# jirsat/wavenets

Measured on AMD Instinct MI355X. Metric: audio samples/sec (training step, 16 kHz mu-law), higher is better.
Workload: dtype f32 (fp16 hi|lo split operands, fp32 accumulate)

## Files before the change

wavenets_amd/csrc/wn_split16.h:

```cpp
#pragma once
#include <hip/hip_fp16.h>

#include "wn_kernels.h"

namespace wn_split16 {

typedef _Float16 h8 __attribute__((ext_vector_type(8)));
typedef _Float16 h4 __attribute__((ext_vector_type(4)));

__device__ __forceinline__ f32x16 mfma16(h8 a, h8 b, f32x16 c) {
  return __builtin_amdgcn_mfma_f32_32x32x16_f16(a, b, c, 0, 0, 0);
}

__device__ __forceinline__ void mfma3(const h8& a_hi, const h8& a_lo, const h8& b_hi, const h8& b_lo, f32x16& acc) {
  acc = mfma16(a_lo, b_hi, acc);
  acc = mfma16(a_hi, b_lo, acc);
  acc = mfma16(a_hi, b_hi, acc);
}

__device__ __forceinline__ void split8(const float (&v)[8], h8& hi, h8& lo) {
#pragma unroll
  for (int e = 0; e < 8; ++e) {
    const _Float16 h = (_Float16)v[e];
    hi[e] = h;
    lo[e] = (_Float16)(v[e] - (float)h);
  }
}
__device__ __forceinline__ void split8(const f32x4& q0, const f32x4& q1, h8& hi, h8& lo) {
  const float v[8] = {q0.x, q0.y, q0.z, q0.w, q1.x, q1.y, q1.z, q1.w};
  split8(v, hi, lo);
}
__device__ __forceinline__ void split4(const f32x4& q, h4& hi, h4& lo) {
  const float v[4] = {q.x, q.y, q.z, q.w};
#pragma unroll
  for (int e = 0; e < 4; ++e) {
    const _Float16 h = (_Float16)v[e];
    hi[e] = h;
    lo[e] = (_Float16)(v[e] - (float)h);
  }
}

__device__ __forceinline__ void split8s(const float (&v)[8], float s, h8& hi, h8& lo) {
#pragma unroll
  for (int e = 0; e < 8; ++e) {
    const _Float16 h = (_Float16)(v[e] * s);
    hi[e] = h;
    lo[e] = (_Float16)__builtin_fmaf(v[e], s, -(float)h);
  }
}
__device__ __forceinline__ void split8s(const f32x4& q0, const f32x4& q1, float s, h8& hi, h8& lo) {
  const float v[8] = {q0.x, q0.y, q0.z, q0.w, q1.x, q1.y, q1.z, q1.w};
  split8s(v, s, hi, lo);
}
__device__ __forceinline__ void split4s(const f32x4& q, float s, h4& hi, h4& lo) {
  const float v[4] = {q.x, q.y, q.z, q.w};
#pragma unroll
  for (int e = 0; e < 4; ++e) {
    const _Float16 h = (_Float16)(v[e] * s);
    hi[e] = h;
    lo[e] = (_Float16)__builtin_fmaf(v[e], s, -(float)h);
  }
}

__device__ __forceinline__ void pow2_scale(float m, float& sc, float& inv) {
  float s = 1.0f, i = 1.0f;
  if (m > 0.f && m < 3.0e38f) {
    int e;
    (void)frexpf(m, &e);
    e = max(-100, min(100, e));
    s = ldexpf(1.0f, -e);
    i = ldexpf(1.0f, e);
  }
  sc = s;
  inv = i;
}

__device__ __forceinline__ f32x4 ldg4(const float* p) { return *(const __attribute__((address_space(1))) f32x4*)(p); }
__device__ __forceinline__ f32x4 ldg4(const __attribute__((address_space(1))) char* p) {
  return *(const __attribute__((address_space(1))) f32x4*)p;
}

__device__ __forceinline__ void dma16(const void* sbase, unsigned voff, unsigned lds_addr) {
  asm volatile("s_mov_b32 m0, %2\n\ts_nop 0\n\tglobal_load_lds_dwordx4 %0, %1"
               :: "v"(voff), "s"(sbase), "s"(lds_addr) : "memory");
}
__device__ __forceinline__ unsigned lds_addr_of(const void* p) {
  return (unsigned)(uintptr_t)(const __attribute__((address_space(3))) unsigned char*)p;
}

template <int PITCH, bool FULL, bool NOSTORE = false, bool ADD = false>
__device__ __forceinline__ void store_tile(const f32x16& v, float* stage, float* dst, unsigned voff, unsigned ld_bytes,
                                           int rows_valid, int lane, const f32x4* add = nullptr) {
  const int tl = lane & 31, h = lane >> 5;
#pragma unroll
  for (int rq = 0; rq < 4; ++rq) {
    f32x4 o;
    o.x = v[4 * rq + 0]; o.y = v[4 * rq + 1]; o.z = v[4 * rq + 2]; o.w = v[4 * rq + 3];
    *reinterpret_cast<f32x4*>(stage + tl * PITCH + 8 * rq + 4 * h) = o;
  }
  asm volatile("s_waitcnt lgkmcnt(0)" ::: "memory");
  const float* rd = stage + (lane >> 3) * PITCH + (lane & 7) * 4;
  char* base0 = reinterpret_cast<char*>(dst);
  asm volatile("" : "+s"(base0));
  __attribute__((address_space(1))) char* base = (__attribute__((address_space(1))) char*)base0;
#pragma unroll
  for (int i = 0; i < 4; ++i) {
    f32x4 o = *reinterpret_cast<const f32x4*>(rd + i * 8 * PITCH);
    if constexpr (ADD) { o.x += add[i].x; o.y += add[i].y; o.z += add[i].z; o.w += add[i].w; }
    if (NOSTORE ? (o.x == 1.2345e-30f) : (FULL || i * 8 + (lane >> 3) < rows_valid))
      *(__attribute__((address_space(1))) f32x4*)(base + (uint64_t)((unsigned)(i * 8) * ld_bytes) + voff) = o;
  }
  asm volatile("" ::: "memory");
}

typedef unsigned u32x4 __attribute__((ext_vector_type(4)));
template <int C32, int PITCH>
__device__ __forceinline__ void wn_store_tile(const f32x16 (&v)[C32], float* stage, float* dst, int ld, int rows_valid, int lane) {
  const int tl = lane & 31, h = lane >> 5;
#pragma unroll
  for (int j = 0; j < C32; ++j)
#pragma unroll
    for (int rq = 0; rq < 4; ++rq) {
      f32x4 o;
      o.x = v[j][4 * rq + 0]; o.y = v[j][4 * rq + 1]; o.z = v[j][4 * rq + 2]; o.w = v[j][4 * rq + 3];
      *reinterpret_cast<f32x4*>(stage + tl * PITCH + 32 * j + 8 * rq + 4 * h) = o;
    }
  asm volatile("s_waitcnt lgkmcnt(0)" ::: "memory");
  constexpr int LPR = C32 * 8;
  constexpr int RPI = 64 / LPR;
  const __amdgpu_buffer_rsrc_t rs = __builtin_amdgcn_make_buffer_rsrc(dst, 0, rows_valid * ld * 4, 0x00020000);
#pragma unroll
  for (int i = 0; i < 32 / RPI; ++i) {
    const int row = i * RPI + lane / LPR;
    const int col = (lane % LPR) * 4;
    const f32x4 o = *reinterpret_cast<const f32x4*>(stage + row * PITCH + col);
    __builtin_amdgcn_raw_buffer_store_b128(__builtin_bit_cast(u32x4, o), rs, (row * ld + col) * 4, 0, 0);
  }
  asm volatile("" ::: "memory");
}

}
```

wavenets_amd/csrc/wn_wgrad_layer.hip:

```cpp
#include "wn_split16.h"

using namespace wn_split16;

template <int C32, bool INNER, bool NO1X1 = false>
__global__ __launch_bounds__(256, 2) void wn_wgrad_layer_kernel(const WnWgLayer* layers, float* ws, float* slab,
                                                                int64_t P, int B, int T, int spb) {
  static_assert(!(INNER && NO1X1), "INNER has no 1x1 part already");
  constexpr bool ONE = !INNER && !NO1X1;
  constexpr int R = 32 * C32, NCH = INNER ? 3 * R : (NO1X1 ? 4 * R : 6 * R);
  constexpr int DUW = INNER ? R : 2 * R;
  constexpr int NXU = ONE ? 2 * 4 * R : 2 * 2 * R;
  constexpr int NU = 1 + (NXU + 255) / 256;
  constexpr int PLANE = NCH * 32;
  constexpr int STAGE = 2 * PLANE;
  constexpr int NJ = INNER ? C32 : ((C32 == 2) ? 4 : 1);
  __shared__ __attribute__((aligned(16))) unsigned char smem[2 * STAGE + 2 * NCH * 4];
  float* bpart = reinterpret_cast<float*>(smem + 2 * STAGE);
  const int tid = threadIdx.x, lane = tid & 63, wave = tid >> 6;
  const int tl = lane & 31, h = lane >> 5;
  const WnWgLayer Ld = layers[blockIdx.y];
  const int split = blockIdx.x;
  const int ub = split / spb, sp = split % spb;
  int len = (T + spb - 1) / spb;
  len = (len + 15) & ~15;
  const int r0 = sp * len, r1 = min(T, r0 + len);
  const int d = Ld.dilation;

  const float* const gmax_u = Ld.gmax_u_off >= 0 ? ws + Ld.gmax_u_off : nullptr;
  const float* const gmax_h = Ld.gmax_h_off >= 0 ? ws + Ld.gmax_h_off : nullptr;
  float su = 1.0f, inv_u = 1.0f, sh = 1.0f, inv_h = 1.0f;
  if (gmax_u) pow2_scale(*gmax_u, su, inv_u);
  if (gmax_h) pow2_scale(*gmax_h, sh, inv_h);

  const float* uptr[NU];
  int ushift[NU], uch[NU], uhh[NU];
  float uscale[NU];
  bool uvalid[NU], ugrad[NU];
  {
    uvalid[0] = tid < 2 * DUW;
    const int c = uvalid[0] ? tid % DUW : 0;
    uch[0] = 2 * R + c;
    uhh[0] = uvalid[0] ? tid / DUW : 0;
    ushift[0] = 0;
    uscale[0] = su;
    ugrad[0] = true;
    uptr[0] = ws + Ld.du_off + (int64_t)ub * T * DUW + c;
  }
#pragma unroll
  for (int i = 1; i < NU; ++i) {
    const int uid = (i - 1) * 256 + tid;
    uvalid[i] = uid < NXU;
    const int c = uvalid[i] ? uid % (NXU / 2) : 0;
    uhh[i] = uvalid[i] ? uid / (NXU / 2) : 0;
    ushift[i] = 0;
    uscale[i] = 1.0f;
    ugrad[i] = false;
    if (c < 2 * R) {
      uch[i] = c;
      uptr[i] = ws + Ld.x_off + (int64_t)ub * T * R + (c % R);
      ushift[i] = c < R ? d : 0;
    } else if (c < 3 * R) {
      uch[i] = 4 * R + (c - 2 * R);
      uptr[i] = ws + Ld.z_off + (int64_t)ub * T * R + (c - 2 * R);
    } else {
      uch[i] = 5 * R + (c - 3 * R);
      uptr[i] = ws + Ld.go_off + (int64_t)ub * T * R + (c - 3 * R);
      uscale[i] = sh;
      ugrad[i] = true;
    }
  }
  float bsum[NU];
#pragma unroll
  for (int i = 0; i < NU; ++i) bsum[i] = 0.f;

  auto load_chunk = [&](int t0, float (&v)[NU][8]) {
    const bool interior = (t0 + 16 <= r1) && (t0 - d >= 0);
    wn_static_for<NU>([&](auto ic) {
      constexpr int i = decltype(ic)::value;
      constexpr int LD = (i == 0) ? DUW : R;
      const int tb = t0 + 8 * uhh[i] - ushift[i];
      const float* p = uptr[i] + (int64_t)tb * LD;
      if (interior && uvalid[i]) {
#pragma unroll
        for (int e = 0; e < 8; ++e) v[i][e] = p[e * LD];
      } else {
#pragma unroll
        for (int e = 0; e < 8; ++e) {
          const bool ok = uvalid[i] && (t0 + 8 * uhh[i] + e < r1) && (tb + e >= 0);
          v[i][e] = ok ? p[e * LD] : 0.f;
        }
      }
    });
  };
  auto store_chunk = [&](int stage, const float (&v)[NU][8]) {
    unsigned char* st = smem + stage * STAGE;
#pragma unroll
    for (int i = 0; i < NU; ++i) {
      if (!uvalid[i]) continue;
      h8 hi, lo;
      float s8 = 0.f;
#pragma unroll
      for (int e = 0; e < 8; ++e) s8 += v[i][e];
      split8s(v[i], uscale[i], hi, lo);
      if (ugrad[i]) bsum[i] += s8;
      *reinterpret_cast<h8*>(st + uch[i] * 32 + uhh[i] * 16) = hi;
      *reinterpret_cast<h8*>(st + PLANE + uch[i] * 32 + uhh[i] * 16) = lo;
    }
  };

  const int xt = (C32 == 2) ? wave : (wave >> 1);
  const int j0 = (C32 == 2 || INNER) ? 0 : (wave & 1);
  const bool has_d = !INNER || C32 == 2 || (wave & 1) == 0;
  const bool has_r = ONE && ((C32 == 2) || wave == 0);
  const int zt = (C32 == 2) ? (wave >> 1) : 0, gt = (C32 == 2) ? (wave & 1) : 0;
  f32x16 acc[NJ], accr;
#pragma unroll
  for (int j = 0; j < NJ; ++j)
#pragma unroll
    for (int r = 0; r < 16; ++r) acc[j][r] = 0.f;
#pragma unroll
  for (int r = 0; r < 16; ++r) accr[r] = 0.f;

  auto compute = [&](int stage) {
    const unsigned char* st = smem + stage * STAGE + tl * 32 + h * 16;
    auto frag = [&](int cb, h8& hi, h8& lo) {
      hi = *reinterpret_cast<const h8*>(st + cb * 32);
      lo = *reinterpret_cast<const h8*>(st + PLANE + cb * 32);
    };
    h8 ah, al;
    if (has_d) frag(32 * xt, ah, al);
#pragma unroll
    for (int j = 0; j < NJ; ++j) {
      if (!has_d) break;
      h8 bh, bl;
      frag(2 * R + 32 * (j0 + j), bh, bl);
      mfma3(ah, al, bh, bl, acc[j]);
    }
    if (has_r) {
      h8 zh, zl, gh, gl;
      frag(4 * R + 32 * zt, zh, zl);
      frag(5 * R + 32 * gt, gh, gl);
      mfma3(zh, zl, gh, gl, accr);
    }
  };

  float va[NU][8], vb[NU][8];
  if (r0 < r1) {
    load_chunk(r0, va);
    if (r0 + 16 < r1) load_chunk(r0 + 16, vb);
    store_chunk(0, va);
  }
  __syncthreads();
  int stage = 0;
  for (int t0 = r0; t0 < r1; t0 += 32) {
    if (t0 + 32 < r1) load_chunk(t0 + 32, va);
    compute(stage);
    if (t0 + 16 < r1) store_chunk(stage ^ 1, vb);
    __syncthreads();
    if (t0 + 16 >= r1) break;
    if (t0 + 48 < r1) load_chunk(t0 + 48, vb);
    compute(stage ^ 1);
    if (t0 + 32 < r1) store_chunk(stage, va);
    __syncthreads();
  }

  float* row = slab + (int64_t)split * P;
  {
    const int tap = xt / C32, kt = xt % C32;
#pragma unroll
    for (int j = 0; j < NJ; ++j)
#pragma unroll
      for (int r = 0; r < 16; ++r) {
        const int k = 32 * kt + wn_drow(r, h);
        if (has_d) row[Ld.dwd_off + ((int64_t)tap * R + k) * DUW + 32 * (j0 + j) + tl] = acc[j][r] * inv_u;
      }
    if (has_r) {
#pragma unroll
      for (int r = 0; r < 16; ++r) {
        const int k = 32 * zt + wn_drow(r, h);
        row[Ld.dwr_off + (int64_t)k * R + 32 * gt + tl] = accr[r] * inv_h;
      }
    }
  }
#pragma unroll
  for (int i = 0; i < NU; ++i)
    if (uvalid[i] && ugrad[i]) bpart[uhh[i] * NCH + uch[i]] = bsum[i];
  __syncthreads();
  for (int c = tid; c < NCH; c += 256) {
    if (c >= 2 * R && c < 2 * R + DUW) { if (Ld.dbd_off >= 0) row[Ld.dbd_off + (c - 2 * R)] = bpart[c] + bpart[NCH + c]; }
    else if (ONE && c >= 5 * R) row[Ld.dbr_off + (c - 5 * R)] = bpart[c] + bpart[NCH + c];
  }
}

int wn_wgrad_layer_supported(int R, int D, int KS) { return R == D && (R == 32 || R == 64) && KS == 2; }

int wn_launch_wgrad_layers(const WnWgLayer* d_layers, int nlayers, int R, float* ws, float* slab, int64_t P, int B,
                           int T, int splits_per_b, hipStream_t s, int inner) {
  if (nlayers <= 0) return WN_OK;
  const dim3 grid((unsigned)(B * splits_per_b), (unsigned)nlayers);
  if (R == 64 && inner == 2) hipLaunchKernelGGL((wn_wgrad_layer_kernel<2, false, true>), grid, dim3(256), 0, s, d_layers, ws, slab, P, B, T, splits_per_b);
  else if (inner == 2) { wn_set_error("wgrad_layers: no form without the 1x1 part at width %d", R); return WN_E_UNSUPPORTED; }
  else if (R == 64 && inner) hipLaunchKernelGGL((wn_wgrad_layer_kernel<2, true>), grid, dim3(256), 0, s, d_layers, ws, slab, P, B, T, splits_per_b);
  else if (R == 32 && inner) hipLaunchKernelGGL((wn_wgrad_layer_kernel<1, true>), grid, dim3(256), 0, s, d_layers, ws, slab, P, B, T, splits_per_b);
  else if (R == 64) hipLaunchKernelGGL((wn_wgrad_layer_kernel<2, false>), grid, dim3(256), 0, s, d_layers, ws, slab, P, B, T, splits_per_b);
  else if (R == 32) hipLaunchKernelGGL((wn_wgrad_layer_kernel<1, false>), grid, dim3(256), 0, s, d_layers, ws, slab, P, B, T, splits_per_b);
  else { wn_set_error("wgrad_layers: unsupported width %d", R); return WN_E_UNSUPPORTED; }
  WN_HIP_CHECK(hipGetLastError());
  return WN_OK;
}
```

wavenets_amd/csrc/wn_wgrad_tr.hip:

```cpp
#include "wn_split16.h"

using namespace wn_split16;

typedef short wt_s4 __attribute__((ext_vector_type(4)));

namespace {

constexpr int WT_ROWS = 32;

template <int PITCH>
__device__ __forceinline__ h8 wt_frag(const unsigned char* lanebase, int off) {
  const wt_s4 a = __builtin_amdgcn_ds_read_tr16_b64_v4i16((__attribute__((address_space(3))) wt_s4*)(lanebase + off));
  const wt_s4 b = __builtin_amdgcn_ds_read_tr16_b64_v4i16((__attribute__((address_space(3))) wt_s4*)(lanebase + off + 4 * PITCH));
  h8 r;
  const h4 ha = *reinterpret_cast<const h4*>(&a), hb = *reinterpret_cast<const h4*>(&b);
  r[0] = ha[0]; r[1] = ha[1]; r[2] = ha[2]; r[3] = ha[3]; r[4] = hb[0]; r[5] = hb[1]; r[6] = hb[2]; r[7] = hb[3];
  return r;
}

}

template <int KC, int NC, int TAPS, int LDX, int LDG, int LDW, int TKW, int TNW, bool G2 = false, int XSEG = 0, bool GSEG = false>
__global__ __launch_bounds__(512, 2) void wn_wgrad_tr_kernel(const WnWgPair* jobs, float* ws, float* slab, int64_t P, int B,
                                                             int T, int spb, float* slab2, int64_t P2) {
  constexpr int XC = TAPS * KC, GC0 = XC + (GSEG ? KC : 0), NCH = GC0 + NC;
  constexpr int PITCH = NCH * 2 + 64;
  constexpr int PLANE = WT_ROWS * PITCH, STAGE = 2 * PLANE;
  constexpr int KT = XC / 32, NT = NC / 32;
  static_assert((KT / TKW) * (NT / TNW) == 8 && KT % TKW == 0 && NT % TNW == 0, "8 waves tile the output block");
  static_assert((PITCH / 4) % 64 == 16, "row pitch must rotate the banks by a quarter");
  static_assert(XSEG == 0 || (TAPS == 1 && !G2 && LDX == XSEG && KC % XSEG == 0 && XSEG % 32 == 0), "segmented X");
  static_assert(!GSEG || (XSEG > 0 && KC == 2 * XSEG && TKW == 1 && NT / TNW == XSEG / 32), "one g_o tile per wave");
  constexpr int XPR = KC / 4, GPR = NC / 4;
  constexpr int XRP = 512 / XPR, GRP = 512 / GPR;
  constexpr int XP = WT_ROWS / XRP, GP = WT_ROWS / GRP;
  constexpr int FBS = GSEG ? WT_ROWS * KC * 4 : 0;
  __shared__ __attribute__((aligned(16))) unsigned char smem[2 * STAGE + 2 * FBS];
  static_assert(2 * STAGE + 2 * FBS <= 160 * 1024 && (GRP * NC + (GSEG ? 2 * KC : 0)) * 4 <= 2 * STAGE, "LDS");
  const int tid = threadIdx.x, lane = tid & 63, wave = __builtin_amdgcn_readfirstlane(tid >> 6);
  const int tl = lane & 31, h = lane >> 5;
  const WnWgPair J = jobs[blockIdx.y];
  const WnWgPair::Seg* const segs = jobs[blockIdx.y].seg;
  const int split = blockIdx.x;
  const int ub = split / spb, sp = split % spb;
  int len = (T + spb - 1) / spb;
  len = (len + WT_ROWS - 1) & ~(WT_ROWS - 1);
  const int r0 = sp * len, r1 = min(T, r0 + len);
  const int d = J.shift;

  float gsc = 1.0f, inv = 1.0f, gsc2 = 1.0f, inv2 = 1.0f;
  if (J.gmax_off >= 0) pow2_scale(ws[J.gmax_off], gsc, inv);
  if constexpr (G2) if (J.gmax2_off >= 0) pow2_scale(ws[J.gmax2_off], gsc2, inv2);

  const int xr = tid / XPR, xc = (tid % XPR) * 4;
  const int gr = tid / GPR, gc = (tid % GPR) * 4;
  const int nseg = XSEG > 0 ? J.nseg : 0;
  const bool xvalid = XSEG == 0 || xc / (XSEG > 0 ? XSEG : 1) < nseg;
  const float* xbase = XSEG > 0 ? ws + J.x_off + (int64_t)(xvalid ? xc / (XSEG > 0 ? XSEG : 1) : 0) * J.seg_stride + (int64_t)ub * T * LDX + xc % (XSEG > 0 ? XSEG : 1)
                                : ws + J.x_off + (int64_t)ub * T * LDX + xc;
  const bool upper = G2 && gc >= NC / 2;
  const float* gbase = upper ? ws + J.g2_off + (int64_t)ub * T * LDG + (gc - NC / 2) : ws + J.g_off + (int64_t)ub * T * LDG + gc;
  const float gs_t = upper ? gsc2 : gsc;
  const int hseg = (GSEG && xvalid) ? xc / (XSEG > 0 ? XSEG : 1) : 0;
  const float* hbase = GSEG ? ws + segs[hseg].g_off + (int64_t)ub * T * XSEG + xc % (XSEG > 0 ? XSEG : 1) : nullptr;
  float hs_t = 1.0f;
  if constexpr (GSEG) {
    float unused;
    if (segs[hseg].gmax_off >= 0) pow2_scale(ws[segs[hseg].gmax_off], hs_t, unused);
  }
  struct Regs { f32x4 xs[TAPS][XP]; f32x4 gv[GP]; f32x4 hv[GSEG ? XP : 1]; };
  Regs ra, rb;
  float bsum[4] = {0.f, 0.f, 0.f, 0.f};
  float hsum = 0.f;
  const f32x4 zero4 = {0.f, 0.f, 0.f, 0.f};

  auto load = [&](int t0, Regs& q) {
    f32x4 (&xs)[TAPS][XP] = q.xs;
    f32x4 (&gv)[GP] = q.gv;
#pragma unroll
    for (int k = 0; k < XP; ++k) {
      const int t = t0 + xr + XRP * k;
      const int tc = min(t, T - 1);
      if (XSEG > 0) {
        xs[0][k] = ldg4(xbase + (int64_t)tc * LDX);
        if constexpr (GSEG) q.hv[k] = ldg4(hbase + (int64_t)tc * XSEG);
      } else {
        xs[0][k] = ldg4(xbase + (int64_t)max(tc - d, 0) * LDX);
        if constexpr (TAPS == 2) xs[1][k] = ldg4(xbase + (int64_t)tc * LDX);
      }
    }
#pragma unroll
    for (int k = 0; k < GP; ++k) {
      const int t = min(t0 + gr + GRP * k, T - 1);
      gv[k] = ldg4(gbase + (int64_t)t * LDG);
    }
  };
  auto store = [&](int stage, const Regs& q, int t0) {
    const f32x4 (&xs)[TAPS][XP] = q.xs;
    const f32x4 (&gv)[GP] = q.gv;
    unsigned char* st = smem + stage * STAGE;
    const bool interior = (t0 + WT_ROWS <= r1) && (t0 - d >= 0);
#pragma unroll
    for (int k = 0; k < XP; ++k) {
      unsigned char* row = st + (xr + XRP * k) * PITCH;
      const int t = t0 + xr + XRP * k;
#pragma unroll
      for (int tp = 0; tp < TAPS; ++tp) {
        h4 hi, lo;
        const bool ok = interior || (t < r1 && (XSEG > 0 || (TAPS == 2 && tp == TAPS - 1) || t - d >= 0));
        const f32x4 xv = (ok && xvalid) ? xs[tp][k] : zero4;
        split4s(xv, 1.0f, hi, lo);
        *reinterpret_cast<h4*>(row + (tp * KC + xc) * 2) = hi;
        *reinterpret_cast<h4*>(row + PLANE + (tp * KC + xc) * 2) = lo;
      }
      if constexpr (GSEG) {
        h4 hi, lo;
        const f32x4 g4 = ((interior || t < r1) && xvalid) ? q.hv[k] : zero4;
        split4s(g4, hs_t, hi, lo);
        *reinterpret_cast<f32x4*>(smem + 2 * STAGE + stage * FBS + ((xr + XRP * k) * KC + xc) * 4) = g4;
        *reinterpret_cast<h4*>(row + (XC + xc) * 2) = hi;
        *reinterpret_cast<h4*>(row + PLANE + (XC + xc) * 2) = lo;
      }
    }
#pragma unroll
    for (int k = 0; k < GP; ++k) {
      h4 hi, lo;
      unsigned char* row = st + (gr + GRP * k) * PITCH;
      const f32x4 g4 = (interior || t0 + gr + GRP * k < r1) ? gv[k] : zero4;
      split4s(g4, gs_t, hi, lo);
      bsum[0] += g4.x; bsum[1] += g4.y; bsum[2] += g4.z; bsum[3] += g4.w;
      *reinterpret_cast<h4*>(row + (GC0 + gc) * 2) = hi;
      *reinterpret_cast<h4*>(row + PLANE + (GC0 + gc) * 2) = lo;
    }
  };

  constexpr int WKD = KT / TKW;
  const int kt0 = TKW * (wave % WKD), nt0 = TNW * (wave / WKD);
  f32x16 acc[TKW][TNW];
#pragma unroll
  for (int i = 0; i < TKW; ++i)
#pragma unroll
    for (int j = 0; j < TNW; ++j)
#pragma unroll
      for (int r = 0; r < 16; ++r) acc[i][j][r] = 0.f;
  const int wseg = GSEG ? 32 * kt0 / (XSEG > 0 ? XSEG : 1) : 0;
  const int ht = wave / WKD;
  f32x16 accr;
#pragma unroll
  for (int r = 0; r < 16; ++r) accr[r] = 0.f;
  const int lb = (8 * h + ((lane & 15) >> 2)) * PITCH + (16 * ((lane >> 4) & 1) + 4 * (lane & 3)) * 2;
  auto compute = [&](int stage) {
    const unsigned char* base = smem + stage * STAGE + lb;
    if constexpr (GSEG) {
      if (wave < 2 * KC / 64) {
        const float* fb = reinterpret_cast<const float*>(smem + 2 * STAGE + stage * FBS) + (8 * (tid / KC)) * KC + tid % KC;
#pragma unroll
        for (int c16 = 0; c16 < WT_ROWS / 16; ++c16) {
          float s8 = 0.f;
#pragma unroll
          for (int e = 0; e < 8; ++e) s8 += fb[(16 * c16 + e) * KC];
          hsum += s8;
        }
      }
    }
    wn_static_for<2>([&](auto kc) {
      constexpr int ks = decltype(kc)::value;
      constexpr int ro = ks * 16 * PITCH;
      h8 ah[TKW], al[TKW];
#pragma unroll
      for (int i = 0; i < TKW; ++i) {
        ah[i] = wt_frag<PITCH>(base, ro + 32 * (kt0 + i) * 2);
        al[i] = wt_frag<PITCH>(base, ro + PLANE + 32 * (kt0 + i) * 2);
      }
#pragma unroll
      for (int j = 0; j < TNW; ++j) {
        const h8 bh = wt_frag<PITCH>(base, ro + (GC0 + 32 * (nt0 + j)) * 2);
        const h8 bl = wt_frag<PITCH>(base, ro + PLANE + (GC0 + 32 * (nt0 + j)) * 2);
#pragma unroll
        for (int i = 0; i < TKW; ++i) {
          mfma3(ah[i], al[i], bh, bl, acc[i][j]);
        }
      }
      if constexpr (GSEG) {
        const h8 bh = wt_frag<PITCH>(base, ro + (XC + XSEG * wseg + 32 * ht) * 2);
        const h8 bl = wt_frag<PITCH>(base, ro + PLANE + (XC + XSEG * wseg + 32 * ht) * 2);
        mfma3(ah[0], al[0], bh, bl, accr);
      }
    });
  };

  constexpr bool DEEP = TAPS == 1;
  if constexpr (DEEP) {
    load(r0, ra);
    load(r0 + WT_ROWS, rb);
    store(0, ra, r0);
    load(r0 + 2 * WT_ROWS, ra);
    __syncthreads();
    for (int t0 = r0; t0 < r1; t0 += 2 * WT_ROWS) {
      store(1, rb, t0 + WT_ROWS);
      load(t0 + 3 * WT_ROWS, rb);
      compute(0);
      __syncthreads();
      if (t0 + WT_ROWS >= r1) break;
      store(0, ra, t0 + 2 * WT_ROWS);
      load(t0 + 4 * WT_ROWS, ra);
      compute(1);
      __syncthreads();
    }
  } else {
    load(r0, ra);
    store(0, ra, r0);
    load(r0 + WT_ROWS, ra);
    __syncthreads();
    int st = 0;
    for (int t0 = r0; t0 < r1; t0 += WT_ROWS, st ^= 1) {
      store(st ^ 1, ra, t0 + WT_ROWS);
      load(t0 + 2 * WT_ROWS, ra);
      compute(st);
      __syncthreads();
    }
  }

  float* row = slab + (int64_t)split * P;
  float* row2 = G2 ? slab2 + (int64_t)split * P2 : nullptr;
#pragma unroll
  for (int i = 0; i < TKW; ++i) {
    if (XSEG > 0 && 32 * (kt0 + i) >= nseg * XSEG) continue;
#pragma unroll
    for (int j = 0; j < TNW; ++j) {
      const int nt = nt0 + j;
      const bool up = G2 && nt >= NT / 2;
      float* tbase = (up ? row2 + J.w2_off + 32 * (nt - NT / 2) : row + J.w_off + 32 * nt) + (int64_t)(32 * (kt0 + i)) * LDW + tl;
      const float iv = up ? inv2 : inv;
#pragma unroll
      for (int r = 0; r < 16; ++r) tbase[wn_drow(r, h) * LDW] = acc[i][j][r] * iv;
    }
  }
  if constexpr (GSEG) {
    if (wseg < nseg) {
      float sc, iv = 1.0f;
      if (segs[wseg].gmax_off >= 0) pow2_scale(ws[segs[wseg].gmax_off], sc, iv);
      float* tbase = slab2 + (int64_t)split * P2 + segs[wseg].w_off + (int64_t)(32 * kt0 - XSEG * wseg) * XSEG + 32 * ht + tl;
#pragma unroll
      for (int r = 0; r < 16; ++r) tbase[wn_drow(r, h) * XSEG] = accr[r] * iv;
    }
    float* hpart = reinterpret_cast<float*>(smem) + GRP * NC;
    if (tid < 2 * KC) hpart[tid] = hsum;
    __syncthreads();
    for (int n = tid; n < KC; n += 512) {
      const int sg = n / (XSEG > 0 ? XSEG : 1);
      if (sg >= nseg || segs[sg].b_off < 0) continue;
      slab2[(int64_t)split * P2 + segs[sg].b_off + n % (XSEG > 0 ? XSEG : 1)] = hpart[n] + hpart[KC + n];
    }
  }
  if (J.b_off >= 0 || (G2 && J.b2_off >= 0)) {
    float* bpart = reinterpret_cast<float*>(smem);
#pragma unroll
    for (int e = 0; e < 4; ++e) bpart[gr * NC + gc + e] = bsum[e];
    __syncthreads();
    for (int n = tid; n < NC; n += 512) {
      float s8 = 0.f;
#pragma unroll
      for (int g = 0; g < GRP; ++g) s8 += bpart[g * NC + n];
      if (G2 && n >= NC / 2) { if (J.b2_off >= 0) row2[J.b2_off + n - NC / 2] = s8; }
      else if (J.b_off >= 0) row[J.b_off + n] = s8;
    }
  }
}

int wn_wgrad_tr_kind(int K, int N, int taps) {
  if (taps == 2) return (K == 128 && N == 256) ? 1 : 0;
  if (K == 128 && N == 128) return 2;
  if (K == 128 && N == 256) return 3;
  if (K == 256 && N == 128) return 4;
  if (K == 256 && N == 256) return 5;
  return 0;
}

int wn_launch_wgrad_tr(int kind, const WnWgPair* d_jobs, int njobs, float* ws, float* slab, int64_t P, int B, int T,
                       int splits_per_b, hipStream_t s, float* slab2, int64_t P2) {
  if (njobs <= 0) return WN_OK;
  const dim3 grid((unsigned)(B * splits_per_b), (unsigned)njobs);
#define WT_LAUNCH(...) hipLaunchKernelGGL((wn_wgrad_tr_kernel<__VA_ARGS__>), grid, dim3(512), 0, s, d_jobs, ws, slab, P, B, T, splits_per_b, slab2, P2)
  switch (kind) {
    case 1: WT_LAUNCH(128, 256, 2, 128, 256, 256, 2, 4); break;
    case 2: WT_LAUNCH(128, 128, 1, 128, 128, 128, 1, 2); break;
    case 3: WT_LAUNCH(128, 256, 1, 128, 256, 256, 1, 4); break;
    case 4: WT_LAUNCH(256, 128, 1, 256, 128, 128, 2, 2); break;
    case 5: WT_LAUNCH(256, 128, 1, 256, 256, 256, 2, 2); break;
    case 6:
      if (!slab2) { wn_set_error("wgrad_tr: kind 6 needs the second slab"); return WN_E_INVALID; }
      WT_LAUNCH(128, 256, 1, 128, 128, 128, 1, 4, true);
      break;
    case 7:
      if (!slab2) { wn_set_error("wgrad_tr: kind 7 needs the second slab"); return WN_E_INVALID; }
      WT_LAUNCH(128, 128, 1, 64, 128, 128, 1, 2, false, 64, true);
      break;
    case 8: WT_LAUNCH(256, 128, 1, 32, 128, 128, 2, 2, false, 32); break;
    default: wn_set_error("wgrad_tr: unknown kind %d", kind); return WN_E_UNSUPPORTED;
  }
#undef WT_LAUNCH
  WN_HIP_CHECK(hipGetLastError());
  return WN_OK;
}
```

Before: 23.93 million.

## Specialize no-1x1 layer wgrad kernel with transposed LDS reads and double buffering

Adds a dedicated specialization of the layer weight-gradient kernel for width 64 without the 1x1 part. It stages split fp16 hi/lo planes of du and shifted x into a padded LDS layout and reads MFMA fragments with ds_read_tr16. Loads are register double-buffered across 32-row chunks so global loads overlap compute. The bias sum is computed during staging. The shared transposed-fragment helper moves into the common header. The generic template now rejects the NO1X1 form, so the specialization carries that path, and its bespoke indexing adds correctness risk.

Result: no change. 24.09 million, median of 4 (+0.7%).

```diff
diff --git a/wavenets_amd/csrc/wn_split16.h b/wavenets_amd/csrc/wn_split16.h
--- a/wavenets_amd/csrc/wn_split16.h
+++ b/wavenets_amd/csrc/wn_split16.h
@@ -80,6 +80,23 @@
   return *(const __attribute__((address_space(1))) f32x4*)p;
 }
 
+typedef short wt_s4 __attribute__((ext_vector_type(4)));
+constexpr int WT_CHUNK_ROWS = 32;
+constexpr bool wt_pitch_ok(int pitch) { return (pitch / 4) % 64 == 16; }
+template <int PITCH>
+__device__ __forceinline__ int wt_lane_base(int lane, int h) {
+  return (8 * h + ((lane & 15) >> 2)) * PITCH + (16 * ((lane >> 4) & 1) + 4 * (lane & 3)) * 2;
+}
+template <int PITCH>
+__device__ __forceinline__ h8 wt_frag(const unsigned char* lanebase, int off) {
+  const wt_s4 a = __builtin_amdgcn_ds_read_tr16_b64_v4i16((__attribute__((address_space(3))) wt_s4*)(lanebase + off));
+  const wt_s4 b = __builtin_amdgcn_ds_read_tr16_b64_v4i16((__attribute__((address_space(3))) wt_s4*)(lanebase + off + 4 * PITCH));
+  h8 r;
+  const h4 ha = *reinterpret_cast<const h4*>(&a), hb = *reinterpret_cast<const h4*>(&b);
+  r[0] = ha[0]; r[1] = ha[1]; r[2] = ha[2]; r[3] = ha[3]; r[4] = hb[0]; r[5] = hb[1]; r[6] = hb[2]; r[7] = hb[3];
+  return r;
+}
+
 __device__ __forceinline__ void dma16(const void* sbase, unsigned voff, unsigned lds_addr) {
   asm volatile("s_mov_b32 m0, %2\n\ts_nop 0\n\tglobal_load_lds_dwordx4 %0, %1"
                :: "v"(voff), "s"(sbase), "s"(lds_addr) : "memory");
diff --git a/wavenets_amd/csrc/wn_wgrad_layer.hip b/wavenets_amd/csrc/wn_wgrad_layer.hip
--- a/wavenets_amd/csrc/wn_wgrad_layer.hip
+++ b/wavenets_amd/csrc/wn_wgrad_layer.hip
@@ -5,9 +5,9 @@
 template <int C32, bool INNER, bool NO1X1 = false>
 __global__ __launch_bounds__(256, 2) void wn_wgrad_layer_kernel(const WnWgLayer* layers, float* ws, float* slab,
                                                                 int64_t P, int B, int T, int spb) {
-  static_assert(!(INNER && NO1X1), "INNER has no 1x1 part already");
-  constexpr bool ONE = !INNER && !NO1X1;
-  constexpr int R = 32 * C32, NCH = INNER ? 3 * R : (NO1X1 ? 4 * R : 6 * R);
+  static_assert(!NO1X1, "the form without the 1x1 part is the specialization wn_wgrad_layer_kernel<2, false, true>");
+  constexpr bool ONE = !INNER;
+  constexpr int R = 32 * C32, NCH = INNER ? 3 * R : 6 * R;
   constexpr int DUW = INNER ? R : 2 * R;
   constexpr int NXU = ONE ? 2 * 4 * R : 2 * 2 * R;
   constexpr int NU = 1 + (NXU + 255) / 256;
@@ -192,6 +192,143 @@
   }
 }
 
+template <>
+__global__ __launch_bounds__(256, 2) void wn_wgrad_layer_kernel<2, false, true>(const WnWgLayer* layers, float* ws, float* slab,
+                                                                                int64_t P, int B, int T, int spb) {
+  constexpr int R = 64, DUW = 2 * R, NCH = 2 * R + DUW;
+  constexpr int PITCH = NCH * 2 + 64;
+  constexpr int PLANE = WT_CHUNK_ROWS * PITCH, STAGE = 2 * PLANE;
+  constexpr int NP = 8;
+  static_assert(wt_pitch_ok(PITCH), "row pitch must rotate the banks by a quarter");
+  static_assert(2 * STAGE <= 80 * 1024 && 2 * DUW * 4 <= STAGE, "two workgroups a CU");
+  __shared__ __attribute__((aligned(16))) unsigned char smem[2 * STAGE];
+  const int tid = threadIdx.x, lane = tid & 63, wave = __builtin_amdgcn_readfirstlane(tid >> 6);
+  const int tl = lane & 31, h = lane >> 5;
+  const WnWgLayer Ld = layers[blockIdx.y];
+  const int split = blockIdx.x;
+  const int ub = split / spb, sp = split % spb;
+  int len = (T + spb - 1) / spb;
+  len = (len + 15) & ~15;
+  const int r0 = sp * len, r1 = min(T, r0 + len);
+  const int d = Ld.dilation;
+  float su = 1.0f, inv_u = 1.0f;
+  if (Ld.gmax_u_off >= 0) pow2_scale(ws[Ld.gmax_u_off], su, inv_u);
+
+  const bool isdu = wave < 2;
+  const int prow = isdu ? 8 * wave + 4 * h : 4 * (wave - 2) + 2 * ((lane >> 4) & 1) + h;
+  const int ra = isdu ? 16 : 0, rb = isdu ? 1 : 8;
+  const int colb = isdu ? (2 * R + 4 * tl) * 2 : 4 * (lane & 15) * 2, ca = isdu ? 0 : R * 2;
+  const int ld = isdu ? DUW : R, sh0 = isdu ? 0 : d;
+  const float scale = isdu ? su : 1.0f;
+  const float* const base = isdu ? ws + Ld.du_off + (int64_t)ub * T * DUW + 4 * tl
+                                 : ws + Ld.x_off + (int64_t)ub * T * R + 4 * (lane & 15);
+  struct Regs { f32x4 v[NP]; };
+  Regs qa, qb;
+  float bsum[4] = {0.f, 0.f, 0.f, 0.f};
+  const f32x4 zero4 = {0.f, 0.f, 0.f, 0.f};
+
+  auto load = [&](int t0, Regs& q) {
+#pragma unroll
+    for (int p = 0; p < NP; ++p) {
+      const int tc = min(t0 + prow + ra * (p >> 2) + rb * (p & 3), r1 - 1);
+      const int ts = max(tc - (p < 4 ? sh0 : 0), 0);
+      q.v[p] = ldg4(base + (int64_t)ts * ld);
+    }
+  };
+  auto store = [&](int stage, const Regs& q, int t0) {
+    unsigned char* st = smem + stage * STAGE + colb;
+    auto piece = [&](int p) {
+      const int t = t0 + prow + ra * (p >> 2) + rb * (p & 3);
+      return (t < r1 && t - (p < 4 ? sh0 : 0) >= 0) ? q.v[p] : zero4;
+    };
+#pragma unroll
+    for (int p = 0; p < NP; ++p) {
+      const int rw = prow + ra * (p >> 2) + rb * (p & 3);
+      h4 hi, lo;
+      split4s(piece(p), scale, hi, lo);
+      *reinterpret_cast<h4*>(st + rw * PITCH + ca * (p >> 2)) = hi;
+      *reinterpret_cast<h4*>(st + PLANE + rw * PITCH + ca * (p >> 2)) = lo;
+    }
+    if (isdu) {
+#pragma unroll
+      for (int ks = 0; ks < 2; ++ks) {
+        f32x4 s = zero4;
+#pragma unroll
+        for (int j = 0; j < 4; ++j) { const f32x4 v = piece(4 * ks + j); s.x += v.x; s.y += v.y; s.z += v.z; s.w += v.w; }
+        f32x4 s8;
+        s8.x = __shfl_xor(s.x, 32); s8.y = __shfl_xor(s.y, 32); s8.z = __shfl_xor(s.z, 32); s8.w = __shfl_xor(s.w, 32);
+#pragma unroll
+        for (int j = 0; j < 4; ++j) { const f32x4 v = piece(4 * ks + j); s8.x += v.x; s8.y += v.y; s8.z += v.z; s8.w += v.w; }
+        bsum[0] += s8.x; bsum[1] += s8.y; bsum[2] += s8.z; bsum[3] += s8.w;
+      }
+    }
+  };
+
+  f32x16 acc[4];
+#pragma unroll
+  for (int j = 0; j < 4; ++j)
+#pragma unroll
+    for (int r = 0; r < 16; ++r) acc[j][r] = 0.f;
+  const int lb = wt_lane_base<PITCH>(lane, h);
+  auto compute = [&](int stage) {
+    const unsigned char* fb = smem + stage * STAGE + lb;
+    wn_static_for<2>([&](auto kc) {
+      constexpr int ro = decltype(kc)::value * 16 * PITCH;
+      const h8 ah = wt_frag<PITCH>(fb, ro + 32 * wave * 2);
+      const h8 al = wt_frag<PITCH>(fb, ro + PLANE + 32 * wave * 2);
+#pragma unroll
+      for (int j = 0; j < 4; ++j) {
+        const h8 bh = wt_frag<PITCH>(fb, ro + (2 * R + 32 * j) * 2);
+        const h8 bl = wt_frag<PITCH>(fb, ro + PLANE + (2 * R + 32 * j) * 2);
+        mfma3(ah, al, bh, bl, acc[j]);
+      }
+    });
+  };
+
+  load(r0, qa);
+  load(r0 + WT_CHUNK_ROWS, qb);
+  store(0, qa, r0);
+  load(r0 + 2 * WT_CHUNK_ROWS, qa);
+  __syncthreads();
+  const int nchunk = (max(r1 - r0, 0) + WT_CHUNK_ROWS - 1) / WT_CHUNK_ROWS;
+  int t0 = r0;
+  for (int i = 0; i + 2 <= nchunk; i += 2, t0 += 2 * WT_CHUNK_ROWS) {
+    store(1, qb, t0 + WT_CHUNK_ROWS);
+    load(t0 + 3 * WT_CHUNK_ROWS, qb);
+    __builtin_amdgcn_sched_barrier(0);
+    compute(0);
+    __syncthreads();
+    store(0, qa, t0 + 2 * WT_CHUNK_ROWS);
+    load(t0 + 4 * WT_CHUNK_ROWS, qa);
+    __builtin_amdgcn_sched_barrier(0);
+    compute(1);
+    __syncthreads();
+  }
+  if (nchunk & 1) {
+    compute(0);
+    __syncthreads();
+  }
+
+  float* row = slab + (int64_t)split * P;
+  {
+    const int tap = wave >> 1, kt = wave & 1;
+#pragma unroll
+    for (int j = 0; j < 4; ++j)
+#pragma unroll
+      for (int r = 0; r < 16; ++r) {
+        const int k = 32 * kt + wn_drow(r, h);
+        row[Ld.dwd_off + ((int64_t)tap * R + k) * DUW + 32 * j + tl] = acc[j][r] * inv_u;
+      }
+  }
+  float* bpart = reinterpret_cast<float*>(smem);
+  if (isdu && h == 1) {
+#pragma unroll
+    for (int e = 0; e < 4; ++e) bpart[wave * DUW + 4 * tl + e] = bsum[e];
+  }
+  __syncthreads();
+  if (tid < DUW && Ld.dbd_off >= 0) row[Ld.dbd_off + tid] = bpart[tid] + bpart[DUW + tid];
+}
+
 int wn_wgrad_layer_supported(int R, int D, int KS) { return R == D && (R == 32 || R == 64) && KS == 2; }
 
 int wn_launch_wgrad_layers(const WnWgLayer* d_layers, int nlayers, int R, float* ws, float* slab, int64_t P, int B,
diff --git a/wavenets_amd/csrc/wn_wgrad_tr.hip b/wavenets_amd/csrc/wn_wgrad_tr.hip
--- a/wavenets_amd/csrc/wn_wgrad_tr.hip
+++ b/wavenets_amd/csrc/wn_wgrad_tr.hip
@@ -2,21 +2,9 @@
 
 using namespace wn_split16;
 
-typedef short wt_s4 __attribute__((ext_vector_type(4)));
-
 namespace {
 
-constexpr int WT_ROWS = 32;
-
-template <int PITCH>
-__device__ __forceinline__ h8 wt_frag(const unsigned char* lanebase, int off) {
-  const wt_s4 a = __builtin_amdgcn_ds_read_tr16_b64_v4i16((__attribute__((address_space(3))) wt_s4*)(lanebase + off));
-  const wt_s4 b = __builtin_amdgcn_ds_read_tr16_b64_v4i16((__attribute__((address_space(3))) wt_s4*)(lanebase + off + 4 * PITCH));
-  h8 r;
-  const h4 ha = *reinterpret_cast<const h4*>(&a), hb = *reinterpret_cast<const h4*>(&b);
-  r[0] = ha[0]; r[1] = ha[1]; r[2] = ha[2]; r[3] = ha[3]; r[4] = hb[0]; r[5] = hb[1]; r[6] = hb[2]; r[7] = hb[3];
-  return r;
-}
+constexpr int WT_ROWS = WT_CHUNK_ROWS;
 
 }
 
@@ -28,7 +16,7 @@
   constexpr int PLANE = WT_ROWS * PITCH, STAGE = 2 * PLANE;
   constexpr int KT = XC / 32, NT = NC / 32;
   static_assert((KT / TKW) * (NT / TNW) == 8 && KT % TKW == 0 && NT % TNW == 0, "8 waves tile the output block");
-  static_assert((PITCH / 4) % 64 == 16, "row pitch must rotate the banks by a quarter");
+  static_assert(wt_pitch_ok(PITCH), "row pitch must rotate the banks by a quarter");
   static_assert(XSEG == 0 || (TAPS == 1 && !G2 && LDX == XSEG && KC % XSEG == 0 && XSEG % 32 == 0), "segmented X");
   static_assert(!GSEG || (XSEG > 0 && KC == 2 * XSEG && TKW == 1 && NT / TNW == XSEG / 32), "one g_o tile per wave");
   constexpr int XPR = KC / 4, GPR = NC / 4;
```
